# AnaryaRay1/naz

Hardware: AMD Instinct MI355X
Metric: samples/sec through log_prob+log|detJ|, 16-dim RQ-spline flow, batch 2^20 (higher is better)
Workload: dtype f32; 1 GPU; BASELINE configs[2]: conditional RQ-spline coupling flow D=16 | C=32, K=8, L=8, H=[128,128], split 8, tanh; fused log_prob (naz_coupling_log_prob); batch_per_gpu=1048576, global_batch=1048576, parallelism=dp1 (independent row shards, no collective)

## Files before the change

### naz_amd/csrc/coupling_r16.h

```cpp
#pragma once
#include "../../include/naz_hip.h"
#include "coupling_x6.h"

namespace naz {

typedef float floatx4 __attribute__((ext_vector_type(4)));

NAZ_DEV floatx4 mfma16_f16(half8 a, half8 b, floatx4 c) { return __builtin_amdgcn_mfma_f32_16x16x32_f16(a, b, c, 0, 0, 0); }
NAZ_DEV floatx4 mfma16_f32(float a, float b, floatx4 c) { return __builtin_amdgcn_mfma_f32_16x16x4f32(a, b, c, 0, 0, 0); }

NAZ_DEV floatx4 mfma3_16(const Frag2& a, const Frag2& b, floatx4 acc) {
  acc = mfma16_f16(a.l, b.h, acc);
  acc = mfma16_f16(a.h, b.l, acc);
  acc = mfma16_f16(a.h, b.h, acc);
  return acc;
}


extern __device__ int64_t g_nonfinite[5];
NAZ_DEV void debug_nonfinite_probe(bool bad, int64_t row, int layer, int stage) {
  if (bad && atomicCAS(reinterpret_cast<unsigned long long*>(&g_nonfinite[0]), 0ull, 1ull) == 0ull) {
    g_nonfinite[1] = blockIdx.x;
    g_nonfinite[2] = layer;
    g_nonfinite[3] = stage;
    g_nonfinite[4] = row;
  }
}

constexpr int kR16Waves = 8;
constexpr int kR16Rows = 16 * kR16Waves;

__host__ __device__ constexpr int r16_feat(int t, int q, int j) { return 32 * t + 16 * (j >> 2) + 4 * q + (j & 3); }

template <int D_, int C_, int S_, int K_, int H_, bool LOWER_>
struct CfgR16 {
  static constexpr int D = D_, C = C_, S = S_, K = K_, H = H_;
  static constexpr bool LOWER = LOWER_;
  static constexpr int Dt = D - S, P = 3 * K - 1, DQ = Dt / 4, SQ = S / 4;
  static constexpr int HB = H / 16;
  static constexpr int KS1 = (C + S + 31) / 32;
  static constexpr int KS2 = H / 32;
  static constexpr int NO = (DQ * P + 3) / 4;
  static constexpr int TBL = 3 * (K + 1);
  static constexpr int OT = 2 * kChunk;
  static constexpr int pad(int n) { return (n + 255) / 256 * 256; }
  static constexpr int pick_kb(int nb, int bias) {
    int best = 1;
    for (int kb = 1; kb <= KS2; ++kb)
      if (KS2 % kb == 0 && pad(nb * kb * OT + bias) <= kX6Slot) best = kb;
    return best;
  }
  static constexpr int KB2 = pick_kb(HB, H), NB2 = KS2 / KB2;
  static constexpr bool SPLIT3 = DQ == 2 && NO % 2 == 0 && (P + 3) / 4 <= NO / 2;
  static constexpr int NOC = SPLIT3 ? NO / 2 : NO;
  static constexpr int KB3 = pick_kb(NOC, 16 * NO), NB3H = KS2 / KB3, NB3 = (SPLIT3 ? 2 : 1) * NB3H;
  static constexpr int C_LAST = C > 32 * (KS1 - 1) ? C - 32 * (KS1 - 1) : 0;
  static constexpr int NR1 = SQ + (C_LAST < 8 - SQ ? C_LAST : 8 - SQ);
  static constexpr bool CAT1 = 3 * NR1 <= 8 && KS1 > 1;
  static constexpr int PC1 = CAT1 ? 2 * KS1 - 1 : 2 * KS1;
  static constexpr __host__ __device__ int g1_pieces(int t) { return CAT1 && t == KS1 - 1 ? 1 : 2; }
  static constexpr int A_BIAS = 0;
  static constexpr int A_TBL = A_BIAS + H;
  static constexpr int A_W = pad(A_TBL + S * TBL);
  static constexpr int A16_SIZE = A_W + HB * PC1 * kChunk;
  static constexpr int A_SIZE = pad(A_W + HB * KS1 * OT);
  static constexpr int B_OFF = A_SIZE;
  static constexpr int B_BIAS = HB * KB2 * OT;
  static constexpr int B_SIZE = pad(B_BIAS + H);
  static constexpr int C_OFF = B_OFF + NB2 * B_SIZE;
  static constexpr int C_BIAS = NOC * KB3 * OT;
  static constexpr int C_SIZE = pad(C_BIAS + 16 * NO);
  static constexpr int A32_OFF = C_OFF + NB3 * C_SIZE;
  static constexpr int LAYER = A32_OFF + A_SIZE;
  static constexpr int NSTG = 1 + NB2 + NB3;
  static constexpr int MAXSTAGE = 2 * kX6Slot;
  static constexpr int SLOT_FREE = kX6Slot - (A_SIZE > B_SIZE ? (A_SIZE > C_SIZE ? A_SIZE : C_SIZE) : (B_SIZE > C_SIZE ? B_SIZE : C_SIZE));
  static constexpr __host__ __device__ int stage_off(int j) {
    return j == 0 ? 0 : (j <= NB2 ? B_OFF + (j - 1) * B_SIZE : C_OFF + (j - 1 - NB2) * C_SIZE);
  }
  static constexpr __host__ __device__ int stage_size(int j) { return j == 0 ? A_SIZE : (j <= NB2 ? B_SIZE : C_SIZE); }
  static constexpr int N_W0 = H * (C + S), N_B0 = H, N_W1 = H * H, N_B1 = H, N_W2 = Dt * P * H, N_B2 = Dt * P;
  static constexpr int N_LOW = LOWER ? S * (3 * K - 1) : 0;
  static constexpr int FLAT = N_W0 + N_B0 + N_W1 + N_B1 + N_W2 + N_B2 + N_LOW;
  static_assert(S % 4 == 0 && Dt % 4 == 0 && H % 32 == 0 && S > 0 && SQ <= 8, "unsupported r16 coupling shape");
  static_assert(A_SIZE <= kX6Slot && B_SIZE <= kX6Slot && C_SIZE <= kX6Slot, "stage exceeds one LDS ring slot");
  static_assert(HB <= 8 && NO <= 16, "register budget");
};

template <class CF>
__host__ __device__ constexpr int r16_in_col(int t, int q, int j) {
  constexpr int TX = CF::KS1 - 1;
  if (t == TX && j < CF::SQ) return CF::C + q * CF::SQ + j;
  int idx = 0;
  if (t < TX) idx = 32 * t + 8 * q + j;
  else idx = 32 * TX + q * (8 - CF::SQ) + (j - CF::SQ);
  return idx < CF::C ? idx : -1;
}

template <class CF>
__host__ __device__ constexpr int r16_out_row(int o, int r) {
  const int q = r >> 2, slot = 4 * o + (r & 3), dq = slot / CF::P, p = slot - dq * CF::P;
  if (dq >= CF::DQ) return -1;
  const int dim = q * CF::DQ + dq;
  if (p < CF::K) return dim * CF::K + p;
  if (p < 2 * CF::K) return CF::Dt * CF::K + dim * CF::K + (p - CF::K);
  return 2 * CF::Dt * CF::K + dim * (CF::K - 1) + (p - 2 * CF::K);
}

template <class CF>
__global__ void coupling_pack_r16_kernel(const float* __restrict__ flat, float* __restrict__ packed, int L,
                                         float bound) {
  const int64_t n = (int64_t)L * CF::LAYER;
  unsigned* pu = reinterpret_cast<unsigned*>(packed);
  for (int64_t e = (int64_t)blockIdx.x * blockDim.x + threadIdx.x; e < n; e += (int64_t)gridDim.x * blockDim.x) {
    const int l = (int)(e / CF::LAYER);
    const int off = (int)(e - (int64_t)l * CF::LAYER);
    const float* W0 = flat + (int64_t)l * CF::FLAT;
    const float* b0 = W0 + CF::N_W0;
    const float* W1 = b0 + CF::N_B0;
    const float* b1 = W1 + CF::N_W1;
    const float* W2 = b1 + CF::N_B1;
    const float* b2 = W2 + CF::N_W2;
    const float* low = b2 + CF::N_B2;
    auto chunk_word = [&](int q, int nt, int t0, int which, int obase = 0) -> unsigned {
      const int o = q / (nt * CF::OT), r1 = q - o * nt * CF::OT;
      const int tl = r1 / CF::OT, r2 = r1 - tl * CF::OT;
      const int piece = r2 / kChunk, u = r2 - piece * kChunk;
      const int lane = u >> 2, pair = u & 3, i = lane & 15, qq = lane >> 4;
      const int t = t0 + tl;
      unsigned out = 0;
      for (int e2 = 0; e2 < 2; ++e2) {
        const int j = 2 * pair + e2;
        float v = 0.f;
        if (which == 1) {
          v = -2.f * kSigScale * W1[(16 * o + i) * CF::H + r16_feat(t, qq, j)];
        } else {
          const int orow = r16_out_row<CF>(obase + o, i);
          v = orow >= 0 ? -2.f * W2[orow * CF::H + r16_feat(t, qq, j)] : 0.f;
        }
        out |= f16_piece_bits(v, piece) << (16 * e2);
      }
      return out;
    };
    unsigned word = 0;
    float fv = 0.f;
    bool is_word = false;
    const bool a32 = off >= CF::A32_OFF;
    if (off < CF::A_SIZE || a32) {
      const int oa = a32 ? off - CF::A32_OFF : off;
      if (oa >= CF::A_W) {
        const int ow = oa - CF::A_W;
        if (!a32) {
          const int o = ow / (CF::PC1 * kChunk), r1 = ow - o * CF::PC1 * kChunk;
          const int pc = r1 / kChunk, u = r1 - pc * kChunk, t = pc >> 1;
          const int lane = u >> 2, pair = u & 3, i = lane & 15, qq = lane >> 4;
          if (o < CF::HB) {
            for (int e2 = 0; e2 < 2; ++e2) {
              int j = 2 * pair + e2, piece = pc & 1;
              bool real = true;
              if (CF::g1_pieces(t) == 1) {
                const int seg = j / CF::NR1;
                j -= seg * CF::NR1;
                piece = seg == 2 ? 1 : 0;
                real = seg < 3;
              }
              const int col = real ? r16_in_col<CF>(t, qq, j) : -1;
              const float v = col >= 0 ? kSigScale * W0[(16 * o + i) * (CF::C + CF::S) + col] : 0.f;
              word |= f16_piece_bits(v, piece) << (16 * e2);
            }
          }
          is_word = true;
        } else if (ow < CF::HB * CF::KS1 * CF::OT) {
          const int i4 = ow & 3, lane = (ow >> 2) & 63, rest = ow >> 8;
          const int s4 = rest % (2 * CF::KS1), o = rest / (2 * CF::KS1);
          const int s = 4 * s4 + i4;
          const int col = r16_in_col<CF>(s / 8, lane >> 4, s % 8);
          fv = col >= 0 ? kSigScale * W0[(16 * o + (lane & 15)) * (CF::C + CF::S) + col] : 0.f;
        }
      } else if (oa < CF::A_TBL) {
        fv = kSigScale * b0[oa - CF::A_BIAS];
      } else if (CF::LOWER && oa < CF::A_TBL + CF::S * CF::TBL) {
        const int q = oa - CF::A_TBL, g = q / CF::TBL, w = q - g * CF::TBL;
        float uw[CF::K], uh[CF::K], ud[CF::K - 1];
        for (int k = 0; k < CF::K; ++k) {
          uw[k] = low[g * CF::K + k];
          uh[k] = low[CF::S * CF::K + g * CF::K + k];
        }
        for (int k = 0; k < CF::K - 1; ++k) ud[k] = low[2 * CF::S * CF::K + g * (CF::K - 1) + k];
        SplineTables<CF::K> tb;
        build_tables<CF::K>(uw, uh, ud, bound, tb);
        const int which = w / (CF::K + 1), k = w - which * (CF::K + 1);
        fv = which == 0 ? tb.cw[k] : (which == 1 ? tb.ch[k] : tb.dv[k]);
      }
    } else if (off < CF::C_OFF) {
      const int sq = (off - CF::B_OFF) / CF::B_SIZE, q = off - CF::B_OFF - sq * CF::B_SIZE;
      if (q < CF::B_BIAS) {
        word = chunk_word(q, CF::KB2, sq * CF::KB2, 1);
        is_word = true;
      } else if (q < CF::B_BIAS + CF::H) {
        fv = kSigScale * b1[q - CF::B_BIAS];
      }
    } else {
      const int sq = (off - CF::C_OFF) / CF::C_SIZE, q = off - CF::C_OFF - sq * CF::C_SIZE;
      if (q < CF::C_BIAS) {
        const int hh = sq / CF::NB3H, s2 = sq - hh * CF::NB3H;
        word = chunk_word(q, CF::KB3, s2 * CF::KB3, 2, hh * CF::NOC);
        is_word = true;
      } else if (q < CF::C_BIAS + 16 * CF::NO) {
        const int r = q - CF::C_BIAS, orow = r16_out_row<CF>(r >> 4, r & 15);
        fv = orow >= 0 ? b2[orow] : 0.f;
      }
    }
    if (is_word) pu[e] = word;
    else packed[e] = fv;
  }
}

template <int NB, int KB, int OB = 0, int NA, class BFn>
NAZ_DEV void gemm_r16_pf(floatx4 (&acc)[NA], const float* __restrict__ stage, int lane, BFn&& bfn) {
  static_assert(OB + NB <= NA, "accumulator window");
  static_assert(2 * NB * KB * 1024 <= 65536, "A fragment offsets must fit the 16-bit LDS offset");
  const unsigned ub = (unsigned)(uintptr_t)to_lds(stage) + 16u * lane;
  auto rd = [&](auto oc, auto tc) {
    constexpr int off = ((decltype(oc)::value * KB + decltype(tc)::value) * 2) * 1024;
    return Frag2{__builtin_bit_cast(half8, lds_read_b128_untracked<off>(ub)),
                 __builtin_bit_cast(half8, lds_read_b128_untracked<off + 1024>(ub))};
  };
  Frag2 an = rd(std::integral_constant<int, 0>{}, std::integral_constant<int, 0>{});
  static_for<0, KB>([&](auto tc) {
    constexpr int t = decltype(tc)::value;
    const Frag2 b = bfn(tc);
    static_for<0, NB>([&](auto oc) {
      constexpr int o = decltype(oc)::value;
      const Frag2 a = an;
      if constexpr (o + 1 < NB || t + 1 < KB) {
        an = rd(std::integral_constant<int, (o + 1 < NB ? o + 1 : 0)>{},
                std::integral_constant<int, (o + 1 < NB ? t : t + 1)>{});
        __builtin_amdgcn_sched_barrier(0);
        lds_wait<2>();
      } else {
        __builtin_amdgcn_sched_barrier(0);
        lds_wait<0>();
      }
      __builtin_amdgcn_sched_barrier(0);
      acc[OB + o] = mfma3_16(a, b, acc[OB + o]);
    });
  });
}

template <class CF>
NAZ_DEV void gemm1_frags(const float (&in)[CF::KS1 * 8], Frag2 (&bf)[CF::KS1]) {
  typedef unsigned short u16x8 __attribute__((ext_vector_type(8)));
#pragma unroll
  for (int t = 0; t < CF::KS1; ++t) {
    float v[8];
#pragma unroll
    for (int jj = 0; jj < 8; ++jj) v[jj] = in[8 * t + jj];
    bf[t] = split8_f16(v);
  }
  if constexpr (CF::CAT1) {
    constexpr int n = CF::NR1;
    const u16x8 h = __builtin_bit_cast(u16x8, bf[CF::KS1 - 1].h), l = __builtin_bit_cast(u16x8, bf[CF::KS1 - 1].l);
    u16x8 c = {0, 0, 0, 0, 0, 0, 0, 0};
#pragma unroll
    for (int j = 0; j < n; ++j) {
      c[j] = h[j];
      c[n + j] = l[j];
      c[2 * n + j] = h[j];
    }
    bf[CF::KS1 - 1].h = __builtin_bit_cast(half8, c);
  }
}

template <class CF, bool PF>
NAZ_DEV void gemm1_r16(floatx4 (&acc)[CF::HB], const float* __restrict__ w, int lane, const Frag2 (&bf)[CF::KS1]) {
  constexpr int HB = CF::HB, KS1 = CF::KS1, PC = CF::PC1;
  if constexpr (PF) {
    static_assert(HB * PC * 1024 <= 65536, "A fragment offsets must fit the 16-bit LDS offset");
    const unsigned ub = (unsigned)(uintptr_t)to_lds(w) + 16u * lane;
    half8 nh, nl = bf[0].l;
    auto rd = [&](auto oc, auto tc) {
      constexpr int t = decltype(tc)::value, off = (decltype(oc)::value * PC + 2 * t) * 1024;
      nh = __builtin_bit_cast(half8, lds_read_b128_untracked<off>(ub));
      if constexpr (CF::g1_pieces(t) == 2) nl = __builtin_bit_cast(half8, lds_read_b128_untracked<off + 1024>(ub));
    };
    rd(std::integral_constant<int, 0>{}, std::integral_constant<int, 0>{});
    static_for<0, KS1>([&](auto tc) {
      constexpr int t = decltype(tc)::value;
      static_for<0, HB>([&](auto oc) {
        constexpr int o = decltype(oc)::value;
        const half8 ah = nh, al = nl;
        if constexpr (o + 1 < HB || t + 1 < KS1) {
          constexpr int t2 = o + 1 < HB ? t : t + 1;
          rd(std::integral_constant<int, (o + 1 < HB ? o + 1 : 0)>{}, std::integral_constant<int, t2>{});
          __builtin_amdgcn_sched_barrier(0);
          lds_wait<CF::g1_pieces(t2)>();
        } else {
          __builtin_amdgcn_sched_barrier(0);
          lds_wait<0>();
        }
        __builtin_amdgcn_sched_barrier(0);
        if constexpr (CF::g1_pieces(t) == 2) acc[o] = mfma3_16(Frag2{ah, al}, bf[t], acc[o]);
        else acc[o] = mfma16_f16(ah, bf[t].h, acc[o]);
      });
    });
  } else {
    const u32x4* c4 = reinterpret_cast<const u32x4*>(w);
#pragma unroll
    for (int t = 0; t < KS1; ++t)
#pragma unroll
      for (int o = 0; o < HB; ++o) {
        const int base = (o * PC + 2 * t) * 64 + lane;
        if (CF::g1_pieces(t) == 2) {
          const Frag2 a{__builtin_bit_cast(half8, c4[base]), __builtin_bit_cast(half8, c4[base + 64])};
          acc[o] = mfma3_16(a, bf[t], acc[o]);
        } else {
          acc[o] = mfma16_f16(__builtin_bit_cast(half8, c4[base]), bf[t].h, acc[o]);
        }
      }
  }
}

template <int NB, int KB, int T0, bool ACT, int NX, bool PF = false>
NAZ_DEV void gemm_r16_lazy(floatx4 (&acc)[NB], const float* __restrict__ stage, int lane, floatx4 (&x)[NX]) {
  if constexpr (PF) {
    gemm_r16_pf<NB, KB>(acc, stage, lane, [&](auto tc) -> Frag2 {
      constexpr int t = decltype(tc)::value;
      float v[8];
#pragma unroll
      for (int j = 0; j < 8; ++j) {
        const int blk = 2 * (T0 + t) + (j >> 2);
        v[j] = blk < NX ? x[blk < NX ? blk : 0][j & 3] : 0.f;
        if constexpr (ACT) v[j] = sig_fold(v[j]);
      }
      return split8_f16(v);
    });
    return;
  }
  const u32x4* c4 = reinterpret_cast<const u32x4*>(stage);
#pragma unroll
  for (int t = 0; t < KB; ++t) {
    float v[8];
#pragma unroll
    for (int j = 0; j < 8; ++j) {
      const int blk = 2 * (T0 + t) + (j >> 2);
      v[j] = blk < NX ? x[blk < NX ? blk : 0][j & 3] : 0.f;
      if constexpr (ACT) v[j] = sig_fold(v[j]);
    }
    const Frag2 b = split8_f16(v);
#pragma unroll
    for (int o = 0; o < NB; ++o) {
      const int base = ((o * KB + t) * 2) * 64 + lane;
      const Frag2 a{__builtin_bit_cast(half8, c4[base]), __builtin_bit_cast(half8, c4[base + 64])};
      acc[o] = mfma3_16(a, b, acc[o]);
    }
  }
}

template <class CF, int s, bool ACT, bool PF = false, int NX>
NAZ_DEV void gemm3_stage(floatx4 (&acc)[CF::NO], const float* __restrict__ cur, int lane, int q, floatx4 (&x)[NX],
                         Frag2 (&f3)[CF::KS2]) {
  constexpr int h = s / CF::NB3H, s2 = s % CF::NB3H, T0 = s2 * CF::KB3, OB = h * CF::NOC;
  if constexpr (s2 == 0) {
    const float4* b4 = reinterpret_cast<const float4*>(cur + CF::C_BIAS);
#pragma unroll
    for (int o = 0; o < CF::NOC; ++o) {
      const float4 bv = b4[4 * (OB + o) + q];
      acc[OB + o] = floatx4{bv.x, bv.y, bv.z, bv.w};
    }
  }
  auto bfrag = [&](auto tc) -> Frag2 {
    constexpr int t = decltype(tc)::value;
    if constexpr (h == 0) {
      float v[8];
#pragma unroll
      for (int j = 0; j < 8; ++j) {
        const int blk = 2 * (T0 + t) + (j >> 2);
        v[j] = blk < NX ? x[blk < NX ? blk : 0][j & 3] : 0.f;
        if constexpr (ACT) v[j] = sig_fold(v[j]);
      }
      f3[T0 + t] = split8_f16(v);
    }
    return f3[T0 + t];
  };
  if constexpr (PF) {
    gemm_r16_pf<CF::NOC, CF::KB3, OB>(acc, cur, lane, bfrag);
    return;
  }
  const u32x4* c4 = reinterpret_cast<const u32x4*>(cur);
  static_for<0, CF::KB3>([&](auto tc) {
    constexpr int t = decltype(tc)::value;
    const Frag2 b = bfrag(tc);
#pragma unroll
    for (int o = 0; o < CF::NOC; ++o) {
      const int base = ((o * CF::KB3 + t) * 2) * 64 + lane;
      const Frag2 a{__builtin_bit_cast(half8, c4[base]), __builtin_bit_cast(half8, c4[base + 64])};
      acc[OB + o] = mfma3_16(a, b, acc[OB + o]);
    }
  });
}

template <class CF, bool DIR_INV, int VAR = 0>
__global__ void __launch_bounds__(kR16Rows * 4, 4) coupling_r16_kernel(
    const float* __restrict__ packed, int L, const float* __restrict__ x, int64_t ldx,
    const float* __restrict__ ctx, int64_t ldc, const float* __restrict__ low, const float* __restrict__ high,
    float* __restrict__ out_lp, float* __restrict__ yout, int64_t ldy, int64_t B, float bound,
    float* __restrict__ states = nullptr, int layer_ld_mode = NAZ_LD_ROWSUM) {
  extern __shared__ float4 lds4[];
  float* const slot0 = reinterpret_cast<float*>(lds4);
  float* const slot1 = slot0 + kX6Slot;
  const int lane = threadIdx.x & 63;
  const int wave = threadIdx.x >> 6;
  const int q = lane >> 4;
  auto tid_now = [&]() {
    int t = threadIdx.x;
    asm volatile("" : "+v"(t));
    return t;
  };
  auto row_of = [&](int t) { return (int64_t)blockIdx.x * kR16Rows + (t >> 6) * 16 + (t & 15); };
  struct Where {
    int64_t row;
    bool valid;
    int q;
  };
  auto where = [&]() {
    const int t = tid_now();
    const int64_t r = row_of(t);
    return Where{r, r < B, (t >> 4) & 3};
  };
  const int64_t row = row_of(threadIdx.x);
  const bool valid = row < B;
  const int64_t crow = valid ? row : 0;

  float zl[CF::SQ], zu[CF::DQ];
  float ldsum = 0.f, logjac = 0.f;
#pragma unroll
  for (int u = 0; u < CF::SQ; ++u) zl[u] = valid ? x[crow * ldx + q * CF::SQ + u] : 0.f;
#pragma unroll
  for (int u = 0; u < CF::DQ; ++u) zu[u] = valid ? x[crow * ldx + CF::S + q * CF::DQ + u] : 0.f;
  if (DIR_INV && low != nullptr) {
    auto bnd = [&](float& v, int dim) {
      const float lo = low[dim], hi = high[dim];
      const float u = (v - lo) / (hi - lo);
      logjac -= logf(u) + log1pf(-u);
      v = logf(u / (1.f - u));
    };
#pragma unroll
    for (int u = 0; u < CF::SQ; ++u) bnd(zl[u], q * CF::SQ + u);
#pragma unroll
    for (int u = 0; u < CF::DQ; ++u) bnd(zu[u], CF::S + q * CF::DQ + u);
    if (q == 0) {
      float sl = 0.f;
      for (int d = 0; d < CF::D; ++d) sl += logf(high[d] - low[d]);
      logjac -= sl;
    }
  }
  constexpr bool kParkLogjac = DIR_INV && VAR != 2 && CF::SLOT_FREE >= kR16Rows * 4;
  if constexpr (kParkLogjac) {
    if (low != nullptr) slot0[kX6Slot - kR16Rows * 4 + threadIdx.x] = logjac;
  }

  bool ok = bound < kG1F16Limit;
#pragma unroll
  for (int u = 0; u < CF::SQ; ++u) ok = ok && fabsf(zl[u]) < kG1F16Limit;
#pragma unroll
  for (int u = 0; u < CF::DQ; ++u) ok = ok && fabsf(zu[u]) < kG1F16Limit;
#pragma unroll
  for (int t = 0; t < CF::KS1; ++t)
#pragma unroll
    for (int j = 0; j < 8; ++j) {
      const int col = r16_in_col<CF>(t, q, j);
      if (col >= 0 && col < CF::C) ok = ok && fabsf(ctx[crow * ldc + col]) < kG1F16Limit;
    }
  {
    int* flags = reinterpret_cast<int*>(slot1);
    if (lane == 0) flags[wave] = __all(ok) ? 1 : 0;
    __syncthreads();
    bool all_ok = true;
#pragma unroll
    for (int w = 0; w < kR16Waves; ++w) all_ok = all_ok && flags[w] != 0;
    ok = all_ok;
  }
  const bool g1f16 = ok;

  const RingSrc ring{packed};
  auto issue_a = [&](float* dst, int l) {
    if (g1f16) stage_issue<CF::A16_SIZE, kR16Waves>(dst, ring, l * CF::LAYER);
    else stage_issue<CF::A_SIZE, kR16Waves>(dst, ring, l * CF::LAYER + CF::A32_OFF);
  };
  issue_a(slot0, DIR_INV ? (L - 1) : 0);

  const RqsConsts<CF::K, DIR_INV> rc(bound);
  float cpre[CF::KS1 * 8];
  auto load_ctx = [&]() {
    const int t_ = tid_now(), q_ = (t_ >> 4) & 3;
    const int64_t r_ = row_of(t_);
    const float* cp = ctx + (r_ < B ? r_ : 0) * ldc;
#pragma unroll
    for (int t = 0; t < CF::KS1; ++t)
#pragma unroll
      for (int jj = 0; jj < 8; ++jj) {
        const int col = r16_in_col<CF>(t, q_, jj);
        cpre[8 * t + jj] = (col >= 0 && col < CF::C) ? cp[col] : 0.f;
      }
  };
  load_ctx();
  int g = 0;
  for (int li = 0; li < L; ++li) {
    const int l = DIR_INV ? (L - 1 - li) : li;
    if constexpr (VAR == 1) {
      const Where w = where();
      if (w.valid) {
        float* st = states + ((int64_t)(l + 1) * B + w.row) * CF::D;
#pragma unroll
        for (int u = 0; u < CF::SQ; ++u) st[w.q * CF::SQ + u] = zl[u];
#pragma unroll
        for (int u = 0; u < CF::DQ; ++u) st[CF::S + w.q * CF::DQ + u] = zu[u];
      }
    }
    floatx4 acc1[CF::HB], acc2[CF::HB], acc3[CF::NO];
    Frag2 f3[CF::KS2];
    auto upper = [&](auto uc) {
      constexpr int u = decltype(uc)::value;
      float uw[CF::K], uh[CF::K], ud[CF::K - 1];
#pragma unroll
      for (int k = 0; k < CF::K; ++k) {
        constexpr int b0 = u * CF::P;
        uw[k] = acc3[(b0 + k) >> 2][(b0 + k) & 3];
        uh[k] = acc3[(b0 + CF::K + k) >> 2][(b0 + CF::K + k) & 3];
      }
#pragma unroll
      for (int k = 0; k < CF::K - 1; ++k) {
        constexpr int b0 = u * CF::P + 2 * CF::K;
        ud[k] = acc3[(b0 + k) >> 2][(b0 + k) & 3];
      }
      float ld;
      zu[u] = rqs_select<CF::K, DIR_INV>(uw, uh, ud, zu[u], bound, rc, ld);
      ldsum += DIR_INV ? -ld : ld;
    };

    static_for<0, CF::NSTG>([&](auto jc) {
      constexpr int j = decltype(jc)::value;
      ring_barrier();
      const float* cur = (g & 1) ? slot1 : slot0;
      float* nxt = (g & 1) ? slot0 : slot1;
      if constexpr (j + 1 < CF::NSTG) {
        stage_issue<CF::stage_size(j + 1), kR16Waves>(nxt, ring, l * CF::LAYER + CF::stage_off(j + 1));
      } else {
        if (li + 1 < L) issue_a(nxt, DIR_INV ? (l - 1) : (l + 1));
      }
      ++g;
      const int lane = tid_now() & 63;

      if constexpr (j == 0) {
#pragma unroll
        for (int u = 0; u < CF::SQ; ++u) {
          if constexpr (DIR_INV && CF::LOWER) {
            float ld;
            zl[u] = rqs_table<CF::K, true>(cur + CF::A_TBL + (q * CF::SQ + u) * CF::TBL, zl[u], bound, ld);
            ldsum -= ld;
          }
        }
        float in[CF::KS1 * 8];
#pragma unroll
        for (int t = 0; t < CF::KS1; ++t)
#pragma unroll
          for (int jj = 0; jj < 8; ++jj) {
            const int col = r16_in_col<CF>(t, q, jj);
            float v = 0.f;
            if (col >= CF::C) v = zl[(col - CF::C - q * CF::SQ) < CF::SQ ? (col - CF::C - q * CF::SQ) : 0];
            else if (col >= 0) v = cpre[8 * t + jj];
            in[8 * t + jj] = v;
          }
        {
          const float4* b4 = reinterpret_cast<const float4*>(cur + CF::A_BIAS);
#pragma unroll
          for (int o = 0; o < CF::HB; ++o) {
            const float4 bv = b4[4 * o + q];
            acc1[o] = floatx4{bv.x, bv.y, bv.z, bv.w};
          }
        }
        if (g1f16) {
          Frag2 bf[CF::KS1];
          gemm1_frags<CF>(in, bf);
          __builtin_amdgcn_s_setprio(1);
          gemm1_r16<CF, true>(acc1, cur + CF::A_W, lane, bf);
          __builtin_amdgcn_s_setprio(0);
        } else {
          const float4* p4 = reinterpret_cast<const float4*>(cur + CF::A_W);
#pragma unroll
          for (int s4 = 0; s4 < 2 * CF::KS1; ++s4)
#pragma unroll
            for (int o = 0; o < CF::HB; ++o) {
              const float4 a = p4[(o * 2 * CF::KS1 + s4) * 64 + lane];
              acc1[o] = mfma16_f32(a.x, in[4 * s4 + 0], acc1[o]);
              acc1[o] = mfma16_f32(a.y, in[4 * s4 + 1], acc1[o]);
              acc1[o] = mfma16_f32(a.z, in[4 * s4 + 2], acc1[o]);
              acc1[o] = mfma16_f32(a.w, in[4 * s4 + 3], acc1[o]);
            }
        }
        if constexpr (!DIR_INV && CF::LOWER) {
#pragma unroll
          for (int u = 0; u < CF::SQ; ++u) {
            float ld;
            zl[u] = rqs_table<CF::K, false>(cur + CF::A_TBL + (q * CF::SQ + u) * CF::TBL, zl[u], bound, ld);
            ldsum += ld;
          }
        }
      } else if constexpr (j <= CF::NB2) {
        constexpr int s = j - 1, T0 = s * CF::KB2;
        if constexpr (s == 0) {
          const float4* b4 = reinterpret_cast<const float4*>(cur + CF::B_BIAS);
#pragma unroll
          for (int o = 0; o < CF::HB; ++o) {
            const float4 bv = b4[4 * o + q];
            acc2[o] = floatx4{bv.x, bv.y, bv.z, bv.w};
          }
        }
        __builtin_amdgcn_s_setprio(1);
        gemm_r16_lazy<CF::HB, CF::KB2, T0, true, CF::HB, true>(acc2, cur, lane, acc1);
        __builtin_amdgcn_s_setprio(0);
      } else {
        constexpr int s = j - 1 - CF::NB2;
        constexpr bool kHost = CF::SPLIT3 && s == CF::NB3H;
        if constexpr (!kHost) __builtin_amdgcn_s_setprio(1);
        gemm3_stage<CF, s, true, true>(acc3, cur, lane, q, acc2, f3);
        if constexpr (!kHost) __builtin_amdgcn_s_setprio(0);
        if constexpr (kHost) upper(std::integral_constant<int, 0>{});
      }
    });

    if (li + 1 < L) load_ctx();
    static_for<CF::SPLIT3 ? 1 : 0, CF::DQ>([&](auto uc) { upper(uc); });
#ifdef NAZ_DEBUG_NONFINITE
    {
      bool fin = isfinite(ldsum);
#pragma unroll
      for (int u = 0; u < CF::SQ; ++u) fin = fin && isfinite(zl[u]);
#pragma unroll
      for (int u = 0; u < CF::DQ; ++u) fin = fin && isfinite(zu[u]);
      debug_nonfinite_probe(valid && !fin, row, li, g);
    }
#endif
  }
  const Where w = where();
  if constexpr (VAR == 1) {
    if (w.valid) {
      float* st = states + w.row * CF::D;
#pragma unroll
      for (int u = 0; u < CF::SQ; ++u) st[w.q * CF::SQ + u] = zl[u];
#pragma unroll
      for (int u = 0; u < CF::DQ; ++u) st[CF::S + w.q * CF::DQ + u] = zu[u];
    }
  }

  if constexpr (VAR == 2) {
    if (w.valid) {
#pragma unroll
      for (int u = 0; u < CF::SQ; ++u) yout[w.row * ldy + w.q * CF::SQ + u] = zl[u];
#pragma unroll
      for (int u = 0; u < CF::DQ; ++u) yout[w.row * ldy + CF::S + w.q * CF::DQ + u] = zu[u];
    }
    float v = ldsum;
    v += __shfl_xor(v, 16);
    v += __shfl_xor(v, 32);
    if (w.q == 0 && w.valid) {
      if (layer_ld_mode == NAZ_LD_ROWSUM_ADD) out_lp[w.row] += v;
      else if (layer_ld_mode == NAZ_LD_ROWSUM_SUB) out_lp[w.row] -= v;
      else out_lp[w.row] = v;
    }
  } else if constexpr (DIR_INV) {
    constexpr float kLogSqrt2Pi = 0.91893853320467274178f;
    float base = 0.f;
#pragma unroll
    for (int u = 0; u < CF::SQ; ++u) base += -(zl[u] * zl[u]) / 2.f - kLogSqrt2Pi;
#pragma unroll
    for (int u = 0; u < CF::DQ; ++u) base += -(zu[u] * zu[u]) / 2.f - kLogSqrt2Pi;
    if constexpr (kParkLogjac) logjac = low != nullptr ? slot0[kX6Slot - kR16Rows * 4 + tid_now()] : 0.f;
    float v = base - ldsum + logjac;
    v += __shfl_xor(v, 16);
    v += __shfl_xor(v, 32);
    if (w.q == 0 && w.valid) out_lp[w.row] = v;
  } else {
    if (low != nullptr) {
#pragma unroll
      for (int u = 0; u < CF::SQ; ++u) {
        const int d = w.q * CF::SQ + u;
        zl[u] = (1.f / (1.f + expf(-zl[u]))) * (high[d] - low[d]) + low[d];
      }
#pragma unroll
      for (int u = 0; u < CF::DQ; ++u) {
        const int d = CF::S + w.q * CF::DQ + u;
        zu[u] = (1.f / (1.f + expf(-zu[u]))) * (high[d] - low[d]) + low[d];
      }
    }
    if (w.valid) {
#pragma unroll
      for (int u = 0; u < CF::SQ; ++u) yout[w.row * ldy + w.q * CF::SQ + u] = zl[u];
#pragma unroll
      for (int u = 0; u < CF::DQ; ++u) yout[w.row * ldy + CF::S + w.q * CF::DQ + u] = zu[u];
    }
    if (out_lp != nullptr) {
      float v = ldsum;
      v += __shfl_xor(v, 16);
      v += __shfl_xor(v, 32);
      if (w.q == 0 && w.valid) out_lp[w.row] = v;
    }
  }
}

}
```

### naz_amd/csrc/lds_ring.h

```cpp
#pragma once
#include "naz_device.h"

namespace naz {

NAZ_DEV __attribute__((address_space(3))) void* to_lds(const void* p) {
  return (__attribute__((address_space(3))) void*)(uint32_t)(uintptr_t)p;
}

typedef unsigned int u32x4_t __attribute__((ext_vector_type(4)));
template <int OFF>
NAZ_DEV u32x4_t lds_read_b128_untracked(unsigned addr) {
  u32x4_t v;
  asm volatile("ds_read_b128 %0, %1 offset:%2" : "=v"(v) : "v"(addr), "i"(OFF));
  return v;
}
template <int N>
NAZ_DEV void lds_wait() {
  __builtin_amdgcn_s_waitcnt(0xC07F | (N << 8));
}

template <int NFLOATS, int NW = 4>
NAZ_DEV void stage_issue(float* lds, const float* __restrict__ src) {
  static_assert(NFLOATS % 256 == 0, "stage must be whole 1 KB chunks");
  constexpr int CHUNKS = NFLOATS / 256;
  const int lane = threadIdx.x & 63;
  const int wave = __builtin_amdgcn_readfirstlane(threadIdx.x >> 6);
#pragma unroll
  for (int c0 = 0; c0 < CHUNKS; c0 += NW) {
    const int c = c0 + wave;
    if (c0 + NW - 1 < CHUNKS || c < CHUNKS) {
      __builtin_amdgcn_global_load_lds(
          (const void __attribute__((address_space(1)))*)(src + c * 256 + lane * 4),
          to_lds(lds + c * 256), 16, 0, 0);
    }
  }
}

struct RingSrc {
  const float* base;
};

template <int NFLOATS, int NW>
NAZ_DEV void stage_issue(float* lds, const RingSrc& src, int off) {
  stage_issue<NFLOATS, NW>(lds, src.base + off);
}

template <int NFLOATS, int NW>
NAZ_DEV void stage_issue_lim(float* lds, const float* __restrict__ src, int nch) {
  static_assert(NFLOATS % 256 == 0, "stage must be whole 1 KB chunks");
  constexpr int CHUNKS = NFLOATS / 256;
  int lane = threadIdx.x & 63;
  asm volatile("" : "+v"(lane));
  const int wave = __builtin_amdgcn_readfirstlane(threadIdx.x >> 6);
  nch = nch < CHUNKS ? nch : CHUNKS;
#pragma unroll
  for (int c0 = 0; c0 < CHUNKS; c0 += NW) {
    const int c = c0 + wave;
    if (c < nch) {
      __builtin_amdgcn_global_load_lds(
          (const void __attribute__((address_space(1)))*)(src + c * 256 + lane * 4),
          to_lds(lds + c * 256), 16, 0, 0);
    }
  }
}

}
```

Measured before the change: 472.7 million samples/s.

## Hoist bias loads to stage start and batch LDS spline-table reads with explicit waits

Bias initialisation for all three GEMMs moves to the top of each ring stage, right after the barrier and before the next stage's prefetch is issued. The lower-half spline table lookup becomes a batched routine that reads the knots of all SQ dimensions with raw ds_read_b32 and immediate offsets, then issues the bin-parameter loads together, so LDS latency overlaps across dimensions. The f32 fallback for GEMM1 now software-pipelines its weight-fragment LDS reads with inline asm and manual waitcnt. The untracked asm loads rely on the manual waits for correctness and limit the compiler's scheduling freedom.

```diff
diff --git a/naz_amd/csrc/coupling_r16.h b/naz_amd/csrc/coupling_r16.h
--- a/naz_amd/csrc/coupling_r16.h
+++ b/naz_amd/csrc/coupling_r16.h
@@ -357,18 +357,63 @@
   }
 }
 
-template <class CF, int s, bool ACT, bool PF = false, int NX>
+template <int NB, int OB = 0, int NA>
+NAZ_DEV void bias_r16(floatx4 (&acc)[NA], const float* __restrict__ bias, int q) {
+  static_assert(OB + NB <= NA, "accumulator window");
+  const float4* b4 = reinterpret_cast<const float4*>(bias);
+#pragma unroll
+  for (int o = 0; o < NB; ++o) {
+    const float4 bv = b4[4 * (OB + o) + q];
+    acc[OB + o] = floatx4{bv.x, bv.y, bv.z, bv.w};
+  }
+}
+
+template <int K, bool INV, int N>
+NAZ_DEV void rqs_table_ring(unsigned tb, float (&z)[N], float bound, float (&ld)[N]) {
+  constexpr int TBL = 3 * (K + 1), SRCH = INV ? K + 1 : 0;
+  static_assert(4 * N * TBL <= 65536, "table offsets must fit the 16-bit LDS offset");
+  float kn[N][K - 1];
+  static_for<0, N>([&](auto uc) {
+    static_for<1, K>([&](auto kc) {
+      constexpr int u = decltype(uc)::value, k = decltype(kc)::value;
+      kn[u][k - 1] = lds_read_b32_untracked<4 * (u * TBL + SRCH + k)>(tb);
+    });
+  });
+  __builtin_amdgcn_sched_barrier(0);
+  lds_wait<0>();
+  __builtin_amdgcn_sched_barrier(0);
+  float v[N][6];
+  static_for<0, N>([&](auto uc) {
+    constexpr int u = decltype(uc)::value;
+    int idx = 0;
+#pragma unroll
+    for (int k = 1; k < K; ++k) idx += (z[u] >= kn[u][k - 1] + kSearchEps) ? 1 : 0;
+    const unsigned at = tb + 4u * (unsigned)idx;
+    v[u][0] = lds_read_b32_untracked<4 * (u * TBL)>(at);
+    v[u][1] = lds_read_b32_untracked<4 * (u * TBL + 1)>(at);
+    v[u][2] = lds_read_b32_untracked<4 * (u * TBL + K + 1)>(at);
+    v[u][3] = lds_read_b32_untracked<4 * (u * TBL + K + 2)>(at);
+    v[u][4] = lds_read_b32_untracked<4 * (u * TBL + 2 * (K + 1))>(at);
+    v[u][5] = lds_read_b32_untracked<4 * (u * TBL + 2 * (K + 1) + 1)>(at);
+  });
+  __builtin_amdgcn_sched_barrier(0);
+  lds_wait<0>();
+  __builtin_amdgcn_sched_barrier(0);
+#pragma unroll
+  for (int u = 0; u < N; ++u) {
+    float lb;
+    const float y = rqs_bin<INV>(z[u], v[u][0], v[u][1] - v[u][0], v[u][2], v[u][3] - v[u][2], v[u][4], v[u][5], lb);
+    const bool inside = z[u] >= -bound && z[u] <= bound;
+    ld[u] = inside ? lb : 0.f;
+    z[u] = inside ? y : z[u];
+  }
+}
+
+template <class CF, int s, bool ACT, bool PF = false, bool BIAS = true, int NX>
 NAZ_DEV void gemm3_stage(floatx4 (&acc)[CF::NO], const float* __restrict__ cur, int lane, int q, floatx4 (&x)[NX],
                          Frag2 (&f3)[CF::KS2]) {
   constexpr int h = s / CF::NB3H, s2 = s % CF::NB3H, T0 = s2 * CF::KB3, OB = h * CF::NOC;
-  if constexpr (s2 == 0) {
-    const float4* b4 = reinterpret_cast<const float4*>(cur + CF::C_BIAS);
-#pragma unroll
-    for (int o = 0; o < CF::NOC; ++o) {
-      const float4 bv = b4[4 * (OB + o) + q];
-      acc[OB + o] = floatx4{bv.x, bv.y, bv.z, bv.w};
-    }
-  }
+  if constexpr (BIAS && s2 == 0) bias_r16<CF::NOC, OB>(acc, cur + CF::C_BIAS, q);
   auto bfrag = [&](auto tc) -> Frag2 {
     constexpr int t = decltype(tc)::value;
     if constexpr (h == 0) {
@@ -544,6 +589,13 @@
       ring_barrier();
       const float* cur = (g & 1) ? slot1 : slot0;
       float* nxt = (g & 1) ? slot0 : slot1;
+      if constexpr (j == 0) {
+        bias_r16<CF::HB>(acc1, cur + CF::A_BIAS, q);
+      } else if constexpr (j == 1) {
+        bias_r16<CF::HB>(acc2, cur + CF::B_BIAS, q);
+      } else if constexpr (j > CF::NB2 && (j - 1 - CF::NB2) % CF::NB3H == 0) {
+        bias_r16<CF::NOC, (j - 1 - CF::NB2) / CF::NB3H * CF::NOC>(acc3, cur + CF::C_BIAS, q);
+      }
       if constexpr (j + 1 < CF::NSTG) {
         stage_issue<CF::stage_size(j + 1), kR16Waves>(nxt, ring, l * CF::LAYER + CF::stage_off(j + 1));
       } else {
@@ -553,13 +605,13 @@
       const int lane = tid_now() & 63;
 
       if constexpr (j == 0) {
-#pragma unroll
-        for (int u = 0; u < CF::SQ; ++u) {
-          if constexpr (DIR_INV && CF::LOWER) {
-            float ld;
-            zl[u] = rqs_table<CF::K, true>(cur + CF::A_TBL + (q * CF::SQ + u) * CF::TBL, zl[u], bound, ld);
-            ldsum -= ld;
-          }
+        [[maybe_unused]] const unsigned tbq =
+            (unsigned)(uintptr_t)to_lds(cur + CF::A_TBL) + 4u * (unsigned)(q * CF::SQ * CF::TBL);
+        if constexpr (DIR_INV && CF::LOWER) {
+          float ld[CF::SQ];
+          rqs_table_ring<CF::K, true>(tbq, zl, bound, ld);
+#pragma unroll
+          for (int u = 0; u < CF::SQ; ++u) ldsum -= ld[u];
         }
         float in[CF::KS1 * 8];
 #pragma unroll
@@ -572,14 +624,6 @@
             else if (col >= 0) v = cpre[8 * t + jj];
             in[8 * t + jj] = v;
           }
-        {
-          const float4* b4 = reinterpret_cast<const float4*>(cur + CF::A_BIAS);
-#pragma unroll
-          for (int o = 0; o < CF::HB; ++o) {
-            const float4 bv = b4[4 * o + q];
-            acc1[o] = floatx4{bv.x, bv.y, bv.z, bv.w};
-          }
-        }
         if (g1f16) {
           Frag2 bf[CF::KS1];
           gemm1_frags<CF>(in, bf);
@@ -587,36 +631,40 @@
           gemm1_r16<CF, true>(acc1, cur + CF::A_W, lane, bf);
           __builtin_amdgcn_s_setprio(0);
         } else {
-          const float4* p4 = reinterpret_cast<const float4*>(cur + CF::A_W);
-#pragma unroll
-          for (int s4 = 0; s4 < 2 * CF::KS1; ++s4)
-#pragma unroll
-            for (int o = 0; o < CF::HB; ++o) {
-              const float4 a = p4[(o * 2 * CF::KS1 + s4) * 64 + lane];
-              acc1[o] = mfma16_f32(a.x, in[4 * s4 + 0], acc1[o]);
-              acc1[o] = mfma16_f32(a.y, in[4 * s4 + 1], acc1[o]);
-              acc1[o] = mfma16_f32(a.z, in[4 * s4 + 2], acc1[o]);
-              acc1[o] = mfma16_f32(a.w, in[4 * s4 + 3], acc1[o]);
-            }
+          constexpr int S4 = 2 * CF::KS1;
+          static_assert(CF::HB * S4 * 1024 <= 65536, "A fragment offsets must fit the 16-bit LDS offset");
+          const unsigned ub = (unsigned)(uintptr_t)to_lds(cur + CF::A_W) + 16u * lane;
+          u32x4_t an = lds_read_b128_untracked<0>(ub);
+          static_for<0, S4>([&](auto sc) {
+            constexpr int s4 = decltype(sc)::value;
+            static_for<0, CF::HB>([&](auto oc) {
+              constexpr int o = decltype(oc)::value;
+              const floatx4 a = __builtin_bit_cast(floatx4, an);
+              if constexpr (o + 1 < CF::HB || s4 + 1 < S4) {
+                constexpr int o2 = o + 1 < CF::HB ? o + 1 : 0, s2 = o + 1 < CF::HB ? s4 : s4 + 1;
+                an = lds_read_b128_untracked<(o2 * S4 + s2) * 1024>(ub);
+                __builtin_amdgcn_sched_barrier(0);
+                lds_wait<1>();
+              } else {
+                __builtin_amdgcn_sched_barrier(0);
+                lds_wait<0>();
+              }
+              __builtin_amdgcn_sched_barrier(0);
+              acc1[o] = mfma16_f32(a[0], in[4 * s4 + 0], acc1[o]);
+              acc1[o] = mfma16_f32(a[1], in[4 * s4 + 1], acc1[o]);
+              acc1[o] = mfma16_f32(a[2], in[4 * s4 + 2], acc1[o]);
+              acc1[o] = mfma16_f32(a[3], in[4 * s4 + 3], acc1[o]);
+            });
+          });
         }
         if constexpr (!DIR_INV && CF::LOWER) {
-#pragma unroll
-          for (int u = 0; u < CF::SQ; ++u) {
-            float ld;
-            zl[u] = rqs_table<CF::K, false>(cur + CF::A_TBL + (q * CF::SQ + u) * CF::TBL, zl[u], bound, ld);
-            ldsum += ld;
-          }
+          float ld[CF::SQ];
+          rqs_table_ring<CF::K, false>(tbq, zl, bound, ld);
+#pragma unroll
+          for (int u = 0; u < CF::SQ; ++u) ldsum += ld[u];
         }
       } else if constexpr (j <= CF::NB2) {
         constexpr int s = j - 1, T0 = s * CF::KB2;
-        if constexpr (s == 0) {
-          const float4* b4 = reinterpret_cast<const float4*>(cur + CF::B_BIAS);
-#pragma unroll
-          for (int o = 0; o < CF::HB; ++o) {
-            const float4 bv = b4[4 * o + q];
-            acc2[o] = floatx4{bv.x, bv.y, bv.z, bv.w};
-          }
-        }
         __builtin_amdgcn_s_setprio(1);
         gemm_r16_lazy<CF::HB, CF::KB2, T0, true, CF::HB, true>(acc2, cur, lane, acc1);
         __builtin_amdgcn_s_setprio(0);
@@ -624,7 +672,7 @@
         constexpr int s = j - 1 - CF::NB2;
         constexpr bool kHost = CF::SPLIT3 && s == CF::NB3H;
         if constexpr (!kHost) __builtin_amdgcn_s_setprio(1);
-        gemm3_stage<CF, s, true, true>(acc3, cur, lane, q, acc2, f3);
+        gemm3_stage<CF, s, true, true, false>(acc3, cur, lane, q, acc2, f3);
         if constexpr (!kHost) __builtin_amdgcn_s_setprio(0);
         if constexpr (kHost) upper(std::integral_constant<int, 0>{});
       }
diff --git a/naz_amd/csrc/lds_ring.h b/naz_amd/csrc/lds_ring.h
--- a/naz_amd/csrc/lds_ring.h
+++ b/naz_amd/csrc/lds_ring.h
@@ -12,6 +12,12 @@
 NAZ_DEV u32x4_t lds_read_b128_untracked(unsigned addr) {
   u32x4_t v;
   asm volatile("ds_read_b128 %0, %1 offset:%2" : "=v"(v) : "v"(addr), "i"(OFF));
+  return v;
+}
+template <int OFF>
+NAZ_DEV float lds_read_b32_untracked(unsigned addr) {
+  float v;
+  asm volatile("ds_read_b32 %0, %1 offset:%2" : "=v"(v) : "v"(addr), "i"(OFF));
   return v;
 }
 template <int N>
```

New measurement: 476.0 million samples/s (median of 6 runs). Within noise of the previous version (+0.7%).
